# Bluear7878/Remote-Sensing-Vision-Language-Diffusion-Model

Measured on NVIDIA B200. Metric: stage2_denoise_steps_per_s_1024sq_cfg2, higher is better.
Workload: dtype bf16

## Files before the change

### remote-sensing-vision-language-diffusion-model_b200/csrc/attention.cu

```cuda
#include "common.cuh"

namespace b200sr {

static constexpr int ATT_BM = 128;
static constexpr int ATT_BN = 128;
static constexpr int ATT_D = 64;
static constexpr int ATT_THREADS = 320;
static constexpr int ATT_STAGES = 2;
static constexpr int ATT_TILE_BYTES = 128 * 64 * 2;
static constexpr int ATT_TMEM_COLS = 256;
static constexpr int ATT_COL_S = 0;
static constexpr int ATT_COL_P = 128;
static constexpr int ATT_COL_O = 192;
static constexpr int ATT_PART_FLOATS = 66 * 128;
static constexpr int ATT_WS_COUNTERS = 512;

struct AttnParams {
  int B, H, Nq, Nk;
  int q_col, k_col, v_col;
  __nv_bfloat16* out;
  long long ldo;
  float scale_log2;
  int causal;
  int n_qtiles, full_ctas, split, blocks_per_split;
  float* partials;
  unsigned int* counters;
#ifdef B200SR_ATT_TRACE
  long long* trace;
#endif
};

#ifdef B200SR_ATT_TRACE
static long long* g_att_trace = nullptr;
#define ATT_T(ev)                                                                                   \
  do {                                                                                              \
    if (p.trace != nullptr && lane == 0 && cta_lin < 4 && j < 64)                                   \
      p.trace[((cta_lin * 10 + warp) * 64 + j) * 8 + (ev)] = clock64();                             \
  } while (0)
__device__ __forceinline__ long long att_gtime() {
  long long t;
  asm volatile("mov.u64 %0, %globaltimer;" : "=l"(t));
  return t;
}
#define ATT_CTA(ev)                                                                                 \
  do {                                                                                              \
    if (p.trace != nullptr && threadIdx.x == 64 && cta_lin < 4096) {                                \
      p.trace[20480 + cta_lin * 3 + (ev)] = att_gtime();                                            \
      if ((ev) == 0) {                                                                              \
        uint32_t smid;                                                                              \
        asm volatile("mov.u32 %0, %smid;" : "=r"(smid));                                            \
        p.trace[20480 + cta_lin * 3 + 2] = smid;                                                    \
      }                                                                                             \
    }                                                                                               \
  } while (0)
#else
#define ATT_T(ev) do { } while (0)
#define ATT_CTA(ev) do { } while (0)
#endif

__device__ __forceinline__ void tmem_st32(uint32_t taddr, const uint32_t (&r)[32]) {
  asm volatile(
      "tcgen05.st.sync.aligned.32x32b.x32.b32 [%0], "
      "{%1, %2, %3, %4, %5, %6, %7, %8, %9, %10, %11, %12, %13, %14, %15, %16, "
      "%17, %18, %19, %20, %21, %22, %23, %24, %25, %26, %27, %28, %29, %30, %31, %32};" ::"r"(taddr),
      "r"(r[0]), "r"(r[1]), "r"(r[2]), "r"(r[3]), "r"(r[4]), "r"(r[5]), "r"(r[6]), "r"(r[7]), "r"(r[8]), "r"(r[9]),
      "r"(r[10]), "r"(r[11]), "r"(r[12]), "r"(r[13]), "r"(r[14]), "r"(r[15]), "r"(r[16]), "r"(r[17]), "r"(r[18]),
      "r"(r[19]), "r"(r[20]), "r"(r[21]), "r"(r[22]), "r"(r[23]), "r"(r[24]), "r"(r[25]), "r"(r[26]), "r"(r[27]),
      "r"(r[28]), "r"(r[29]), "r"(r[30]), "r"(r[31])
      : "memory");
}

__device__ __forceinline__ float ex2_approx(float x) {
  float y;
  asm("ex2.approx.ftz.f32 %0, %1;" : "=f"(y) : "f"(x));
  return y;
}

__global__ void __launch_bounds__(ATT_THREADS, 2)
attention_d64_kernel(const __grid_constant__ CUtensorMap tmQ, const __grid_constant__ CUtensorMap tmK,
                     const __grid_constant__ CUtensorMap tmV, const AttnParams p) {
  extern __shared__ __align__(1024) uint8_t smem_raw[];
  uint8_t* smem = reinterpret_cast<uint8_t*>((reinterpret_cast<uintptr_t>(smem_raw) + 1023) & ~uintptr_t(1023));
  uint8_t* sQ = smem;
  uint8_t* sKV = smem + ATT_TILE_BYTES;
  uint64_t* bars = reinterpret_cast<uint64_t*>(sKV + ATT_STAGES * 2 * ATT_TILE_BYTES);
  uint64_t* q_full = bars;
  uint64_t* kv_full = bars + 1;
  uint64_t* kv_empty = kv_full + ATT_STAGES;
  uint64_t* s_full = kv_empty + ATT_STAGES;
  uint64_t* p_full = s_full + 1;
  uint64_t* o_done = p_full + 1;
  uint32_t* tmem_slot = reinterpret_cast<uint32_t*>(o_done + 1);
  float* s_xch = reinterpret_cast<float*>(tmem_slot + 2);

  const int warp = threadIdx.x >> 5, lane = threadIdx.x & 31;
  int tile = blockIdx.x, jb0 = 0, split_idx = -1, tail_idx = 0;
  int nblk = (p.Nk + ATT_BN - 1) / ATT_BN;
  if (static_cast<int>(blockIdx.x) >= p.full_ctas) {
    const int t = blockIdx.x - p.full_ctas;
    tail_idx = t / p.split;
    split_idx = t - tail_idx * p.split;
    tile = p.full_ctas + tail_idx;
    jb0 = split_idx * p.blocks_per_split;
    nblk = min(nblk - jb0, p.blocks_per_split);
  }
  const int q0 = (tile % p.n_qtiles) * ATT_BM;
  const int h = (tile / p.n_qtiles) % p.H, b = tile / (p.n_qtiles * p.H);
#ifdef B200SR_ATT_TRACE
  const int cta_lin = blockIdx.x;
#endif
  ATT_CTA(0);

  if (warp == 0 && lane == 0) {
    tma_prefetch_desc(&tmQ);
    tma_prefetch_desc(&tmK);
    tma_prefetch_desc(&tmV);
    mbar_init(q_full, 1);
    for (int s = 0; s < ATT_STAGES; ++s) {
      mbar_init(&kv_full[s], 1);
      mbar_init(&kv_empty[s], 1);
    }
    mbar_init(s_full, 1);
    mbar_init(p_full, 8);
    mbar_init(o_done, 1);
    fence_barrier_init();
  }
  if (warp == 1) {
    tmem_alloc(tmem_slot, ATT_TMEM_COLS);
    tmem_relinquish();
  }
  tc_fence_before();
  __syncthreads();
  tc_fence_after();
  const uint32_t tmem = *tmem_slot;
  pdl_launch_dependents();

  if (warp == 0) {
    if (lane == 0) {
      pdl_wait();
      mbar_expect_tx(q_full, ATT_TILE_BYTES);
      tma_load_3d(sQ, &tmQ, q_full, p.q_col + h * ATT_D, q0, b);
      int stage = 0;
      uint32_t phase = 0;
      for (int j = 0; j < nblk; ++j) {
        mbar_wait(&kv_empty[stage], phase ^ 1);
        ATT_T(0);
        uint8_t* sK = sKV + stage * 2 * ATT_TILE_BYTES;
        uint8_t* sV = sK + ATT_TILE_BYTES;
        mbar_expect_tx(&kv_full[stage], 2 * ATT_TILE_BYTES);
        tma_load_3d(sK, &tmK, &kv_full[stage], p.k_col + h * ATT_D, (jb0 + j) * ATT_BN, b);
        tma_load_3d(sV, &tmV, &kv_full[stage], p.v_col + h * ATT_D, (jb0 + j) * ATT_BN, b);
        if (++stage == ATT_STAGES) {
          stage = 0;
          phase ^= 1;
        }
      }
    }
  } else if (warp == 1) {
    if (lane == 0) {
      const uint32_t idesc_s = umma_idesc_bf16_f32(ATT_BM, ATT_BN, 0, 0);
      const uint32_t idesc_o = umma_idesc_bf16_f32(ATT_BM, ATT_D, 0, 1);
      const uint64_t qdesc = umma_smem_desc_sw128(smem_u32(sQ), 16, 1024);
      mbar_wait(q_full, 0);
      int stage = 0;
      uint32_t phase = 0;
      mbar_wait(&kv_full[0], 0);
      tc_fence_after();
      {
        const uint64_t kdesc = umma_smem_desc_sw128(smem_u32(sKV), 16, 1024);
#pragma unroll
        for (int k = 0; k < ATT_D / 16; ++k) umma_ss(tmem + ATT_COL_S, qdesc + 2 * k, kdesc + 2 * k, idesc_s, k != 0);
        umma_commit(s_full);
      }
      for (int j = 0; j < nblk; ++j) {
        mbar_wait(p_full, j & 1);
        ATT_T(0);
        tc_fence_after();
        {
          const uint32_t sV = smem_u32(sKV + stage * 2 * ATT_TILE_BYTES + ATT_TILE_BYTES);
          const uint64_t vdesc = umma_smem_desc_sw128(sV, 1024, 1024);
#pragma unroll
          for (int k = 0; k < ATT_BN / 16; ++k) {
            umma_ts(tmem + ATT_COL_O, tmem + ATT_COL_P + 8 * k, vdesc + (2048 >> 4) * k, idesc_o, (j | k) != 0);
          }
          umma_commit(&kv_empty[stage]);
          if (j + 1 == nblk) umma_commit(o_done);
        }
        ATT_T(1);
        if (++stage == ATT_STAGES) {
          stage = 0;
          phase ^= 1;
        }
        if (j + 1 < nblk) {
          mbar_wait(&kv_full[stage], phase);
          ATT_T(2);
          tc_fence_after();
          const uint64_t kdesc = umma_smem_desc_sw128(smem_u32(sKV + stage * 2 * ATT_TILE_BYTES), 16, 1024);
#pragma unroll
          for (int k = 0; k < ATT_D / 16; ++k)
            umma_ss(tmem + ATT_COL_S, qdesc + 2 * k, kdesc + 2 * k, idesc_s, k != 0);
          umma_commit(s_full);
          ATT_T(3);
        }
      }
    }
  } else {
    const int sub = warp & 3;
    const int half = (warp - 2) >> 2;
    const int r = sub * 32 + lane;
    const uint32_t lane_base = static_cast<uint32_t>(sub * 32) << 16;
    float m_used = -INFINITY;
    float l = 0.f;
    for (int j = 0; j < nblk; ++j) {
      mbar_wait(s_full, j & 1);
      ATT_T(0);
      tc_fence_after();
      float s[64];
#pragma unroll
      for (int c = 0; c < 2; ++c) {
        uint32_t a[32];
        tmem_ld32(tmem + lane_base + ATT_COL_S + half * 64 + c * 32, a);
#pragma unroll
        for (int i = 0; i < 32; ++i) s[c * 32 + i] = __uint_as_float(a[i]);
      }
      tmem_ld_wait();
      ATT_T(1);
      int kv_left = p.Nk - (jb0 + j) * ATT_BN - half * 64;
      if (p.causal) kv_left = min(kv_left, q0 + r + 1 - (jb0 + j) * ATT_BN - half * 64);
      if (kv_left < 64) {
#pragma unroll
        for (int i = 0; i < 64; ++i)
          if (i >= kv_left) s[i] = -INFINITY;
      }
      float mx = s[0];
#pragma unroll
      for (int i = 1; i < 64; ++i) mx = fmaxf(mx, s[i]);
      float* xch = s_xch + (j & 1) * 256;
      xch[half * 128 + r] = mx;
      asm volatile("bar.sync 1, 256;" ::: "memory");
      ATT_T(2);
      mx = fmaxf(mx, xch[(half ^ 1) * 128 + r]) * p.scale_log2;
      const bool grow = mx > m_used + 8.0f;
      if (j == 0) {
        m_used = mx;
      } else if (__any_sync(0xffffffffu, grow)) {
        float alpha = 1.0f;
        if (grow) {
          alpha = ex2_approx(m_used - mx);
          m_used = mx;
          l *= alpha;
        }
        uint32_t o[32];
        tmem_ld32(tmem + lane_base + ATT_COL_O + half * 32, o);
        tmem_ld_wait();
#pragma unroll
        for (int i = 0; i < 32; ++i) o[i] = __float_as_uint(__uint_as_float(o[i]) * alpha);
        tmem_st32(tmem + lane_base + ATT_COL_O + half * 32, o);
      }
      float sum0 = 0.f, sum1 = 0.f;
      uint32_t pk[32];
#pragma unroll
      for (int i = 0; i < 32; ++i) {
        const float e0 = ex2_approx(fmaf(s[2 * i], p.scale_log2, -m_used));
        const float e1 = ex2_approx(fmaf(s[2 * i + 1], p.scale_log2, -m_used));
        sum0 += e0;
        sum1 += e1;
        pk[i] = pack_bf16x2(e0, e1);
      }
      ATT_T(3);
      tmem_st32(tmem + lane_base + ATT_COL_P + half * 32, pk);
      l += sum0 + sum1;
      tmem_st_wait();
      ATT_T(4);
      tc_fence_before();
      __syncwarp();
      if (lane == 0) mbar_arrive(p_full);
      ATT_T(5);
    }
    float* xch = s_xch + (nblk & 1) * 256;
    xch[half * 128 + r] = l;
    asm volatile("bar.sync 1, 256;" ::: "memory");
    l += xch[(half ^ 1) * 128 + r];
    mbar_wait(o_done, 0);
    tc_fence_after();
    const int q = q0 + r;
    uint32_t o[32];
    tmem_ld32(tmem + lane_base + ATT_COL_O + half * 32, o);
    tmem_ld_wait();
    bool write_out = true;
    if (split_idx >= 0) {
      float* part = p.partials + (static_cast<size_t>(tail_idx) * p.split + split_idx) * ATT_PART_FLOATS;
#pragma unroll
      for (int i = 0; i < 32; ++i) part[(half * 32 + i) * 128 + r] = __uint_as_float(o[i]);
      if (half == 0) {
        part[64 * 128 + r] = m_used;
        part[65 * 128 + r] = l;
      }
      __threadfence();
      asm volatile("bar.sync 1, 256;" ::: "memory");
      if (threadIdx.x == 64) {
        const unsigned int prev = atomicAdd(&p.counters[tail_idx], 1u);
        tmem_slot[1] = (prev == static_cast<unsigned int>(p.split) - 1u) ? 1u : 0u;
        __threadfence();
      }
      asm volatile("bar.sync 1, 256;" ::: "memory");
      write_out = tmem_slot[1] != 0u;
      if (write_out) {
        const float* base = p.partials + static_cast<size_t>(tail_idx) * p.split * ATT_PART_FLOATS;
        float m_all = -INFINITY;
        for (int s2 = 0; s2 < p.split; ++s2) m_all = fmaxf(m_all, __ldcg(base + s2 * ATT_PART_FLOATS + 64 * 128 + r));
        float acc[32];
#pragma unroll
        for (int i = 0; i < 32; ++i) acc[i] = 0.f;
        l = 0.f;
        for (int s2 = 0; s2 < p.split; ++s2) {
          const float* ps = base + s2 * ATT_PART_FLOATS;
          const float w = ex2_approx(__ldcg(ps + 64 * 128 + r) - m_all);
          l = fmaf(w, __ldcg(ps + 65 * 128 + r), l);
#pragma unroll
          for (int i = 0; i < 32; ++i) acc[i] = fmaf(w, __ldcg(ps + (half * 32 + i) * 128 + r), acc[i]);
        }
#pragma unroll
        for (int i = 0; i < 32; ++i) o[i] = __float_as_uint(acc[i]);
        if (threadIdx.x == 64) p.counters[tail_idx] = 0u;
      }
    }
    const float inv_l = 1.0f / l;
    if (write_out && q < p.Nq) {
      __nv_bfloat16* dst = p.out + (static_cast<long long>(b) * p.Nq + q) * p.ldo + h * ATT_D + half * 32;
#pragma unroll
      for (int v = 0; v < 4; ++v) {
        uint4 u;
        u.x = pack_bf16x2(__uint_as_float(o[v * 8 + 0]) * inv_l, __uint_as_float(o[v * 8 + 1]) * inv_l);
        u.y = pack_bf16x2(__uint_as_float(o[v * 8 + 2]) * inv_l, __uint_as_float(o[v * 8 + 3]) * inv_l);
        u.z = pack_bf16x2(__uint_as_float(o[v * 8 + 4]) * inv_l, __uint_as_float(o[v * 8 + 5]) * inv_l);
        u.w = pack_bf16x2(__uint_as_float(o[v * 8 + 6]) * inv_l, __uint_as_float(o[v * 8 + 7]) * inv_l);
        reinterpret_cast<uint4*>(dst)[v] = u;
      }
    }
  }

  ATT_CTA(1);
  tc_fence_before();
  __syncthreads();
  tc_fence_after();
  if (warp == 1) tmem_dealloc(tmem, ATT_TMEM_COLS);
}

static int make_map3(CUtensorMap* m, const void* base, long long ld, int rows, int batch, int width_cols) {
  uint64_t dims[3] = {static_cast<uint64_t>(width_cols), static_cast<uint64_t>(rows), static_cast<uint64_t>(batch)};
  uint64_t strides[2] = {static_cast<uint64_t>(ld) * 2, static_cast<uint64_t>(rows) * ld * 2};
  uint32_t box[3] = {ATT_D, 128, 1};
  return make_tmap_bf16(m, base, 3, dims, strides, box);
}

struct AttnPlan {
  int n_qtiles, tiles, full, tail, split, blocks_per_split;
  size_t workspace_bytes;
};

static AttnPlan attention_plan(int B, int H, int Nq, int Nk) {
  AttnPlan a;
  a.n_qtiles = (Nq + ATT_BM - 1) / ATT_BM;
  a.tiles = B * H * a.n_qtiles;
  const int nblk = (Nk + ATT_BN - 1) / ATT_BN;
  const int slots = 2 * num_sms();
  a.split = 1;
  a.blocks_per_split = nblk;
  a.full = a.tiles;
  a.tail = 0;
  if (slots <= 0) {
    a.workspace_bytes = 0;
    return a;
  }
  a.full = (a.tiles / slots) * slots;
  a.tail = a.tiles - a.full;
  if (a.tail > 0 && a.tail <= ATT_WS_COUNTERS) {
    int s = 1;
    while (s * 2 <= nblk && a.tail * s * 2 <= slots && s * 2 <= 4) s *= 2;
    if (s > 1) {
      a.blocks_per_split = (nblk + s - 1) / s;
      a.split = (nblk + a.blocks_per_split - 1) / a.blocks_per_split;
    }
  }
  if (a.split == 1) {
    a.full = a.tiles;
    a.tail = 0;
  }
  a.workspace_bytes = a.tail == 0 ? 0
                                  : ATT_WS_COUNTERS * sizeof(unsigned int) +
                                        static_cast<size_t>(a.tail) * a.split * ATT_PART_FLOATS * sizeof(float);
  return a;
}

size_t attention_d64_workspace_bytes(int B, int H, int Nq, int Nk) {
  if (B <= 0 || H <= 0 || Nq <= 0 || Nk <= 0) return 0;
  return attention_plan(B, H, Nq, Nk).workspace_bytes;
}

int attention_d64(const void* q, long long ldq, int q_col, const void* k, long long ldk, int k_col, const void* v,
                  long long ldv, int v_col, void* out, long long ldo, int B, int H, int Nq, int Nk, float scale,
                  int causal, void* workspace, cudaStream_t stream) {
  if (B <= 0 || H <= 0 || Nq <= 0 || Nk <= 0) return B200SR_EINVAL;
  if (causal && (Nq != Nk || Nk > ATT_BN)) return B200SR_EINVAL;
  if ((ldq % 8) || (ldk % 8) || (ldv % 8) || (ldo % 8) || (q_col % 8) || (k_col % 8) || (v_col % 8))
    return B200SR_EINVAL;
  if (q_col + H * ATT_D > ldq || k_col + H * ATT_D > ldk || v_col + H * ATT_D > ldv || H * ATT_D > ldo)
    return B200SR_EINVAL;
  const AttnPlan plan = attention_plan(B, H, Nq, Nk);
  if (plan.workspace_bytes != 0 && workspace == nullptr) return B200SR_EINVAL;
  CUtensorMap tmQ, tmK, tmV;
  int rc = make_map3(&tmQ, q, ldq, Nq, B, static_cast<int>(ldq));
  if (rc) return rc;
  rc = make_map3(&tmK, k, ldk, Nk, B, static_cast<int>(ldk));
  if (rc) return rc;
  rc = make_map3(&tmV, v, ldv, Nk, B, static_cast<int>(ldv));
  if (rc) return rc;
  AttnParams p;
  p.B = B;
  p.H = H;
  p.Nq = Nq;
  p.Nk = Nk;
  p.q_col = q_col;
  p.k_col = k_col;
  p.v_col = v_col;
  p.out = reinterpret_cast<__nv_bfloat16*>(out);
  p.ldo = ldo;
  p.scale_log2 = scale * 1.4426950408889634f;
  p.causal = causal;
  p.n_qtiles = plan.n_qtiles;
  p.full_ctas = plan.full;
  p.split = plan.split;
  p.blocks_per_split = plan.blocks_per_split;
  p.counters = reinterpret_cast<unsigned int*>(workspace);
  p.partials = reinterpret_cast<float*>(reinterpret_cast<unsigned int*>(workspace) + ATT_WS_COUNTERS);
#ifdef B200SR_ATT_TRACE
  p.trace = g_att_trace;
#endif
  const size_t smem_bytes = ATT_TILE_BYTES * (1 + 2 * ATT_STAGES) + 1024 + 128 + 2048;
  static bool attr_set[64] = {false};
  if (first_use_on_device(attr_set)) {
    if (cudaFuncSetAttribute(attention_d64_kernel, cudaFuncAttributeMaxDynamicSharedMemorySize,
                             static_cast<int>(smem_bytes)) != cudaSuccess)
      return B200SR_ELAUNCH;
  }
  dim3 grid(plan.full + plan.tail * plan.split);
  return launch_k(attention_d64_kernel, grid, dim3(ATT_THREADS), smem_bytes, stream, 1, tmQ, tmK, tmV, p) == cudaSuccess
             ? B200SR_OK
             : B200SR_ELAUNCH;
}

}

#ifdef B200SR_ATT_TRACE
extern "C" void b200sr_debug_set_attn_trace(void* p) { b200sr::g_att_trace = reinterpret_cast<long long*>(p); }
#endif
```

Measured before the change: 38.20.

## Process two Q tiles per CTA with ping-pong softmax and shared K/V stages

Each CTA now handles a pair of adjacent 128-row query tiles that share every K/V block. Each tile gets its own 256-column TMEM region and its own 4-warp softmax group, and a polling MMA issuer interleaves QK and PV for both units so one unit's tensor-core work overlaps the other's softmax. K/V staging grows to three stages and the cross-half max exchange through shared memory is removed, since each thread now owns a full 128-wide row. The kernel drops to one CTA per SM with 512 TMEM columns, so it loses inter-CTA overlap, risks register pressure from the 128-float row, and the grid shrinks, which may hurt tail balance.

```diff
diff --git a/remote-sensing-vision-language-diffusion-model_b200/csrc/attention.cu b/remote-sensing-vision-language-diffusion-model_b200/csrc/attention.cu
--- a/remote-sensing-vision-language-diffusion-model_b200/csrc/attention.cu
+++ b/remote-sensing-vision-language-diffusion-model_b200/csrc/attention.cu
@@ -6,9 +6,10 @@
 static constexpr int ATT_BN = 128;
 static constexpr int ATT_D = 64;
 static constexpr int ATT_THREADS = 320;
-static constexpr int ATT_STAGES = 2;
+static constexpr int ATT_STAGES = 3;
 static constexpr int ATT_TILE_BYTES = 128 * 64 * 2;
-static constexpr int ATT_TMEM_COLS = 256;
+static constexpr int ATT_TMEM_COLS = 512;
+static constexpr int ATT_UNIT_COLS = 256;
 static constexpr int ATT_COL_S = 0;
 static constexpr int ATT_COL_P = 128;
 static constexpr int ATT_COL_O = 192;
@@ -22,7 +23,7 @@
   long long ldo;
   float scale_log2;
   int causal;
-  int n_qtiles, full_ctas, split, blocks_per_split;
+  int n_qtiles, full_tiles, tiles, full_ctas, split, blocks_per_split;
   float* partials;
   unsigned int* counters;
 #ifdef B200SR_ATT_TRACE
@@ -30,12 +31,44 @@
 #endif
 };
 
+__host__ __device__ inline int att_pairs(int lo, int hi, int nq) {
+  if (lo >= hi) return 0;
+  const int head_end = (lo / nq + 1) * nq;
+  const int a0 = (hi < head_end ? hi : head_end) - lo;
+  const int rest = hi - lo - a0;
+  return (a0 + 1) / 2 + (rest / nq) * ((nq + 1) / 2) + (rest % nq + 1) / 2;
+}
+__device__ __forceinline__ int att_pair_at(int c, int lo, int hi, int nq, bool& has1) {
+  const int a0 = min(hi, (lo / nq + 1) * nq) - lo;
+  const int c0 = (a0 + 1) / 2;
+  int t, head_end;
+  if (c < c0) {
+    t = lo + 2 * c;
+    head_end = lo + a0;
+  } else {
+    c -= c0;
+    const int cph = (nq + 1) / 2;
+    const int g = c / cph;
+    t = lo + a0 + g * nq + 2 * (c - g * cph);
+    head_end = min(hi, lo + a0 + (g + 1) * nq);
+  }
+  has1 = t + 1 < head_end;
+  return t;
+}
+
 #ifdef B200SR_ATT_TRACE
 static long long* g_att_trace = nullptr;
+static constexpr int ATT_TRACE_EV = 16;
+static constexpr int ATT_TRACE_CTA_OFF = 4 * 10 * 64 * ATT_TRACE_EV;
 #define ATT_T(ev)                                                                                   \
   do {                                                                                              \
     if (p.trace != nullptr && lane == 0 && cta_lin < 4 && j < 64)                                   \
-      p.trace[((cta_lin * 10 + warp) * 64 + j) * 8 + (ev)] = clock64();                             \
+      p.trace[((cta_lin * 10 + warp) * 64 + j) * ATT_TRACE_EV + (ev)] = clock64();                  \
+  } while (0)
+#define ATT_TV(ev, val)                                                                             \
+  do {                                                                                              \
+    if (p.trace != nullptr && lane == 0 && cta_lin < 4 && j < 64)                                   \
+      p.trace[((cta_lin * 10 + warp) * 64 + j) * ATT_TRACE_EV + (ev)] = (val);                      \
   } while (0)
 __device__ __forceinline__ long long att_gtime() {
   long long t;
@@ -45,17 +78,25 @@
 #define ATT_CTA(ev)                                                                                 \
   do {                                                                                              \
     if (p.trace != nullptr && threadIdx.x == 64 && cta_lin < 4096) {                                \
-      p.trace[20480 + cta_lin * 3 + (ev)] = att_gtime();                                            \
+      p.trace[ATT_TRACE_CTA_OFF + cta_lin * 3 + (ev)] = att_gtime();                                \
       if ((ev) == 0) {                                                                              \
         uint32_t smid;                                                                              \
         asm volatile("mov.u32 %0, %smid;" : "=r"(smid));                                            \
-        p.trace[20480 + cta_lin * 3 + 2] = smid;                                                    \
+        p.trace[ATT_TRACE_CTA_OFF + cta_lin * 3 + 2] = smid;                                        \
       }                                                                                             \
     }                                                                                               \
   } while (0)
+#define ATT_MMA_ISSUE(stmt)                                                                         \
+  do {                                                                                              \
+    const long long t_i = clock64();                                                                \
+    stmt;                                                                                           \
+    busy += clock64() - t_i;                                                                        \
+  } while (0)
 #else
 #define ATT_T(ev) do { } while (0)
+#define ATT_TV(ev, val) do { } while (0)
 #define ATT_CTA(ev) do { } while (0)
+#define ATT_MMA_ISSUE(stmt) stmt
 #endif
 
 __device__ __forceinline__ void tmem_st32(uint32_t taddr, const uint32_t (&r)[32]) {
@@ -76,36 +117,48 @@
   return y;
 }
 
-__global__ void __launch_bounds__(ATT_THREADS, 2)
+__device__ __forceinline__ void bar_sync_unit(int u) {
+  if (u == 0)
+    asm volatile("bar.sync 1, 128;" ::: "memory");
+  else
+    asm volatile("bar.sync 2, 128;" ::: "memory");
+}
+
+__global__ void __launch_bounds__(ATT_THREADS, 1)
 attention_d64_kernel(const __grid_constant__ CUtensorMap tmQ, const __grid_constant__ CUtensorMap tmK,
                      const __grid_constant__ CUtensorMap tmV, const AttnParams p) {
   extern __shared__ __align__(1024) uint8_t smem_raw[];
   uint8_t* smem = reinterpret_cast<uint8_t*>((reinterpret_cast<uintptr_t>(smem_raw) + 1023) & ~uintptr_t(1023));
   uint8_t* sQ = smem;
-  uint8_t* sKV = smem + ATT_TILE_BYTES;
+  uint8_t* sKV = smem + 2 * ATT_TILE_BYTES;
   uint64_t* bars = reinterpret_cast<uint64_t*>(sKV + ATT_STAGES * 2 * ATT_TILE_BYTES);
   uint64_t* q_full = bars;
   uint64_t* kv_full = bars + 1;
   uint64_t* kv_empty = kv_full + ATT_STAGES;
   uint64_t* s_full = kv_empty + ATT_STAGES;
-  uint64_t* p_full = s_full + 1;
-  uint64_t* o_done = p_full + 1;
-  uint32_t* tmem_slot = reinterpret_cast<uint32_t*>(o_done + 1);
-  float* s_xch = reinterpret_cast<float*>(tmem_slot + 2);
+  uint64_t* s_free = s_full + 2;
+  uint64_t* p_full = s_free + 2;
+  uint64_t* pv_done = p_full + 2;
+  uint32_t* tmem_slot = reinterpret_cast<uint32_t*>(pv_done + 2);
+  uint32_t* last_flag = tmem_slot + 1;
 
   const int warp = threadIdx.x >> 5, lane = threadIdx.x & 31;
-  int tile = blockIdx.x, jb0 = 0, split_idx = -1, tail_idx = 0;
+  bool has1;
+  int tile0, jb0 = 0, split_idx = -1;
   int nblk = (p.Nk + ATT_BN - 1) / ATT_BN;
-  if (static_cast<int>(blockIdx.x) >= p.full_ctas) {
-    const int t = blockIdx.x - p.full_ctas;
-    tail_idx = t / p.split;
-    split_idx = t - tail_idx * p.split;
-    tile = p.full_ctas + tail_idx;
+  if (static_cast<int>(blockIdx.x) < p.full_ctas) {
+    tile0 = att_pair_at(blockIdx.x, 0, p.full_tiles, p.n_qtiles, has1);
+  } else {
+    const int c = blockIdx.x - p.full_ctas;
+    const int pair = c / p.split;
+    split_idx = c - pair * p.split;
+    tile0 = att_pair_at(pair, p.full_tiles, p.tiles, p.n_qtiles, has1);
     jb0 = split_idx * p.blocks_per_split;
     nblk = min(nblk - jb0, p.blocks_per_split);
   }
-  const int q0 = (tile % p.n_qtiles) * ATT_BM;
-  const int h = (tile / p.n_qtiles) % p.H, b = tile / (p.n_qtiles * p.H);
+  const int nunits = has1 ? 2 : 1;
+  const int q00 = (tile0 % p.n_qtiles) * ATT_BM;
+  const int h = (tile0 / p.n_qtiles) % p.H, b = tile0 / (p.n_qtiles * p.H);
 #ifdef B200SR_ATT_TRACE
   const int cta_lin = blockIdx.x;
 #endif
@@ -120,9 +173,12 @@
       mbar_init(&kv_full[s], 1);
       mbar_init(&kv_empty[s], 1);
     }
-    mbar_init(s_full, 1);
-    mbar_init(p_full, 8);
-    mbar_init(o_done, 1);
+    for (int u = 0; u < 2; ++u) {
+      mbar_init(&s_full[u], 1);
+      mbar_init(&s_free[u], 4);
+      mbar_init(&p_full[u], 4);
+      mbar_init(&pv_done[u], 1);
+    }
     fence_barrier_init();
   }
   if (warp == 1) {
@@ -138,13 +194,13 @@
   if (warp == 0) {
     if (lane == 0) {
       pdl_wait();
-      mbar_expect_tx(q_full, ATT_TILE_BYTES);
-      tma_load_3d(sQ, &tmQ, q_full, p.q_col + h * ATT_D, q0, b);
+      mbar_expect_tx(q_full, nunits * ATT_TILE_BYTES);
+      for (int u = 0; u < nunits; ++u)
+        tma_load_3d(sQ + u * ATT_TILE_BYTES, &tmQ, q_full, p.q_col + h * ATT_D, q00 + u * ATT_BM, b);
       int stage = 0;
       uint32_t phase = 0;
       for (int j = 0; j < nblk; ++j) {
         mbar_wait(&kv_empty[stage], phase ^ 1);
-        ATT_T(0);
         uint8_t* sK = sKV + stage * 2 * ATT_TILE_BYTES;
         uint8_t* sV = sK + ATT_TILE_BYTES;
         mbar_expect_tx(&kv_full[stage], 2 * ATT_TILE_BYTES);
@@ -160,182 +216,235 @@
     if (lane == 0) {
       const uint32_t idesc_s = umma_idesc_bf16_f32(ATT_BM, ATT_BN, 0, 0);
       const uint32_t idesc_o = umma_idesc_bf16_f32(ATT_BM, ATT_D, 0, 1);
-      const uint64_t qdesc = umma_smem_desc_sw128(smem_u32(sQ), 16, 1024);
+#ifdef B200SR_ATT_TRACE
+      long long busy = 0;
+#endif
+      auto issue_qk = [&](int u, int stage) {
+        const uint64_t qdesc = umma_smem_desc_sw128(smem_u32(sQ + u * ATT_TILE_BYTES), 16, 1024);
+        const uint64_t kdesc = umma_smem_desc_sw128(smem_u32(sKV + stage * 2 * ATT_TILE_BYTES), 16, 1024);
+#pragma unroll
+        for (int k = 0; k < ATT_D / 16; ++k)
+          umma_ss(tmem + u * ATT_UNIT_COLS + ATT_COL_S, qdesc + 2 * k, kdesc + 2 * k, idesc_s, k != 0);
+        umma_commit(&s_full[u]);
+      };
+      auto issue_pv = [&](int u, int stage, int j) {
+        const uint64_t vdesc =
+            umma_smem_desc_sw128(smem_u32(sKV + stage * 2 * ATT_TILE_BYTES + ATT_TILE_BYTES), 1024, 1024);
+        const uint32_t tu = tmem + u * ATT_UNIT_COLS;
+#pragma unroll
+        for (int k = 0; k < ATT_BN / 16; ++k) {
+          umma_ts(tu + ATT_COL_O, tu + ATT_COL_P + 8 * k, vdesc + (2048 >> 4) * k, idesc_o, (j | k) != 0);
+        }
+        umma_commit(&pv_done[u]);
+      };
       mbar_wait(q_full, 0);
-      int stage = 0;
-      uint32_t phase = 0;
       mbar_wait(&kv_full[0], 0);
       tc_fence_after();
-      {
-        const uint64_t kdesc = umma_smem_desc_sw128(smem_u32(sKV), 16, 1024);
-#pragma unroll
-        for (int k = 0; k < ATT_D / 16; ++k) umma_ss(tmem + ATT_COL_S, qdesc + 2 * k, kdesc + 2 * k, idesc_s, k != 0);
-        umma_commit(s_full);
-      }
-      for (int j = 0; j < nblk; ++j) {
-        mbar_wait(p_full, j & 1);
-        ATT_T(0);
-        tc_fence_after();
-        {
-          const uint32_t sV = smem_u32(sKV + stage * 2 * ATT_TILE_BYTES + ATT_TILE_BYTES);
-          const uint64_t vdesc = umma_smem_desc_sw128(sV, 1024, 1024);
-#pragma unroll
-          for (int k = 0; k < ATT_BN / 16; ++k) {
-            umma_ts(tmem + ATT_COL_O, tmem + ATT_COL_P + 8 * k, vdesc + (2048 >> 4) * k, idesc_o, (j | k) != 0);
+      for (int u = 0; u < nunits; ++u) issue_qk(u, 0);
+      int qk_next[2] = {1, 1}, pv_next[2] = {0, 0};
+      if (nunits == 1) qk_next[1] = pv_next[1] = nblk;
+      int kv_ready = 1, freed = 0;
+#if B200SR_HANG_GUARD
+      long long t_idle = 0;
+      uint32_t idle = 0;
+#endif
+      while (freed < nblk) {
+        bool progress = false;
+        if (kv_ready < nblk && mbar_test_wait(&kv_full[kv_ready % ATT_STAGES], (kv_ready / ATT_STAGES) & 1)) {
+          const int j = kv_ready;
+          ATT_T(0);
+          ++kv_ready;
+          progress = true;
+        }
+#pragma unroll
+        for (int u = 0; u < 2; ++u) {
+          const int jp = pv_next[u];
+          if (jp < qk_next[u] && mbar_test_wait(&p_full[u], jp & 1)) {
+            tc_fence_after();
+            ATT_MMA_ISSUE(issue_pv(u, jp % ATT_STAGES, jp));
+            const int j = jp;
+            ATT_T(2 + 2 * u);
+            pv_next[u] = jp + 1;
+            progress = true;
           }
-          umma_commit(&kv_empty[stage]);
-          if (j + 1 == nblk) umma_commit(o_done);
-        }
-        ATT_T(1);
-        if (++stage == ATT_STAGES) {
-          stage = 0;
-          phase ^= 1;
-        }
-        if (j + 1 < nblk) {
-          mbar_wait(&kv_full[stage], phase);
-          ATT_T(2);
-          tc_fence_after();
-          const uint64_t kdesc = umma_smem_desc_sw128(smem_u32(sKV + stage * 2 * ATT_TILE_BYTES), 16, 1024);
-#pragma unroll
-          for (int k = 0; k < ATT_D / 16; ++k)
-            umma_ss(tmem + ATT_COL_S, qdesc + 2 * k, kdesc + 2 * k, idesc_s, k != 0);
-          umma_commit(s_full);
-          ATT_T(3);
-        }
+          const int jq = qk_next[u];
+          if (jq < kv_ready && mbar_test_wait(&s_free[u], (jq - 1) & 1)) {
+            tc_fence_after();
+            ATT_MMA_ISSUE(issue_qk(u, jq % ATT_STAGES));
+            const int j = jq;
+            ATT_T(1 + 2 * u);
+            qk_next[u] = jq + 1;
+            progress = true;
+          }
+        }
+        while (freed < min(pv_next[0], pv_next[1])) {
+          umma_commit(&kv_empty[freed % ATT_STAGES]);
+          const int j = freed;
+          ATT_T(5);
+          ATT_TV(8, busy);
+          ++freed;
+          progress = true;
+        }
+#if B200SR_HANG_GUARD
+        if (progress) {
+          idle = 0;
+        } else if (++idle == 1024u) {
+          t_idle = clock64();
+        } else if (idle > 1024u && (idle & 1023u) == 0 && clock64() - t_idle > 8000000000LL) {
+          __trap();
+        }
+#endif
       }
     }
   } else {
-    const int sub = warp & 3;
-    const int half = (warp - 2) >> 2;
-    const int r = sub * 32 + lane;
-    const uint32_t lane_base = static_cast<uint32_t>(sub * 32) << 16;
-    float m_used = -INFINITY;
-    float l = 0.f;
-    for (int j = 0; j < nblk; ++j) {
-      mbar_wait(s_full, j & 1);
-      ATT_T(0);
+    const int u = (warp - 2) >> 2;
+    const int quad = warp & 3;
+    const int r = quad * 32 + lane;
+    const uint32_t tu = tmem + (static_cast<uint32_t>(quad * 32) << 16) + u * ATT_UNIT_COLS;
+    const int q0 = q00 + u * ATT_BM;
+    if (u < nunits) {
+      float m_used = -INFINITY;
+      float l = 0.f;
+      for (int j = 0; j < nblk; ++j) {
+        mbar_wait(&s_full[u], j & 1);
+        ATT_T(0);
+        tc_fence_after();
+        float s[128];
+#pragma unroll
+        for (int c = 0; c < 4; ++c) {
+          uint32_t a[32];
+          tmem_ld32(tu + ATT_COL_S + c * 32, a);
+#pragma unroll
+          for (int i = 0; i < 32; ++i) s[c * 32 + i] = __uint_as_float(a[i]);
+        }
+        tmem_ld_wait();
+        tc_fence_before();
+        __syncwarp();
+        if (lane == 0) mbar_arrive(&s_free[u]);
+        ATT_T(1);
+        int kv_left = p.Nk - (jb0 + j) * ATT_BN;
+        if (p.causal) kv_left = min(kv_left, q0 + r + 1 - (jb0 + j) * ATT_BN);
+        if (kv_left < ATT_BN) {
+#pragma unroll
+          for (int i = 0; i < ATT_BN; ++i)
+            if (i >= kv_left) s[i] = -INFINITY;
+        }
+        float mx0 = s[0], mx1 = s[1], mx2 = s[2], mx3 = s[3];
+#pragma unroll
+        for (int i = 4; i < ATT_BN; i += 4) {
+          mx0 = fmaxf(mx0, s[i]);
+          mx1 = fmaxf(mx1, s[i + 1]);
+          mx2 = fmaxf(mx2, s[i + 2]);
+          mx3 = fmaxf(mx3, s[i + 3]);
+        }
+        const float mx = fmaxf(fmaxf(mx0, mx1), fmaxf(mx2, mx3)) * p.scale_log2;
+        ATT_T(2);
+        const bool grow = mx > m_used + 8.0f;
+        const bool rescale = j != 0 && __any_sync(0xffffffffu, grow);
+        float alpha = 1.0f;
+        if (j == 0) {
+          m_used = mx;
+        } else {
+          if (grow) {
+            alpha = ex2_approx(m_used - mx);
+            m_used = mx;
+            l *= alpha;
+          }
+          mbar_wait(&pv_done[u], (j - 1) & 1);
+          tc_fence_after();
+        }
+        ATT_T(3);
+        float sum[4] = {0.f, 0.f, 0.f, 0.f};
+#pragma unroll
+        for (int c = 0; c < 4; ++c) {
+          uint32_t pk[16];
+#pragma unroll
+          for (int i = 0; i < 16; ++i) {
+            const float e0 = ex2_approx(fmaf(s[c * 32 + 2 * i], p.scale_log2, -m_used));
+            const float e1 = ex2_approx(fmaf(s[c * 32 + 2 * i + 1], p.scale_log2, -m_used));
+            sum[(c >> 1) * 2] += e0;
+            sum[(c >> 1) * 2 + 1] += e1;
+            pk[i] = pack_bf16x2(e0, e1);
+          }
+          tmem_st16(tu + ATT_COL_P + c * 16, pk);
+        }
+        l += (sum[0] + sum[1]) + (sum[2] + sum[3]);
+        if (rescale) {
+#pragma unroll
+          for (int c = 0; c < 2; ++c) {
+            uint32_t o[32];
+            tmem_ld32(tu + ATT_COL_O + c * 32, o);
+            tmem_ld_wait();
+#pragma unroll
+            for (int i = 0; i < 32; ++i) o[i] = __float_as_uint(__uint_as_float(o[i]) * alpha);
+            tmem_st32(tu + ATT_COL_O + c * 32, o);
+          }
+        }
+        ATT_T(4);
+        tmem_st_wait();
+        tc_fence_before();
+        __syncwarp();
+        if (lane == 0) mbar_arrive(&p_full[u]);
+        ATT_T(5);
+      }
+      mbar_wait(&pv_done[u], (nblk - 1) & 1);
       tc_fence_after();
-      float s[64];
+      const int q = q0 + r;
+      float o[64];
 #pragma unroll
       for (int c = 0; c < 2; ++c) {
         uint32_t a[32];
-        tmem_ld32(tmem + lane_base + ATT_COL_S + half * 64 + c * 32, a);
-#pragma unroll
-        for (int i = 0; i < 32; ++i) s[c * 32 + i] = __uint_as_float(a[i]);
+        tmem_ld32(tu + ATT_COL_O + c * 32, a);
+        tmem_ld_wait();
+#pragma unroll
+        for (int i = 0; i < 32; ++i) o[c * 32 + i] = __uint_as_float(a[i]);
       }
-      tmem_ld_wait();
-      ATT_T(1);
-      int kv_left = p.Nk - (jb0 + j) * ATT_BN - half * 64;
-      if (p.causal) kv_left = min(kv_left, q0 + r + 1 - (jb0 + j) * ATT_BN - half * 64);
-      if (kv_left < 64) {
-#pragma unroll
-        for (int i = 0; i < 64; ++i)
-          if (i >= kv_left) s[i] = -INFINITY;
-      }
-      float mx = s[0];
-#pragma unroll
-      for (int i = 1; i < 64; ++i) mx = fmaxf(mx, s[i]);
-      float* xch = s_xch + (j & 1) * 256;
-      xch[half * 128 + r] = mx;
-      asm volatile("bar.sync 1, 256;" ::: "memory");
-      ATT_T(2);
-      mx = fmaxf(mx, xch[(half ^ 1) * 128 + r]) * p.scale_log2;
-      const bool grow = mx > m_used + 8.0f;
-      if (j == 0) {
-        m_used = mx;
-      } else if (__any_sync(0xffffffffu, grow)) {
-        float alpha = 1.0f;
-        if (grow) {
-          alpha = ex2_approx(m_used - mx);
-          m_used = mx;
-          l *= alpha;
-        }
-        uint32_t o[32];
-        tmem_ld32(tmem + lane_base + ATT_COL_O + half * 32, o);
-        tmem_ld_wait();
-#pragma unroll
-        for (int i = 0; i < 32; ++i) o[i] = __float_as_uint(__uint_as_float(o[i]) * alpha);
-        tmem_st32(tmem + lane_base + ATT_COL_O + half * 32, o);
-      }
-      float sum0 = 0.f, sum1 = 0.f;
-      uint32_t pk[32];
-#pragma unroll
-      for (int i = 0; i < 32; ++i) {
-        const float e0 = ex2_approx(fmaf(s[2 * i], p.scale_log2, -m_used));
-        const float e1 = ex2_approx(fmaf(s[2 * i + 1], p.scale_log2, -m_used));
-        sum0 += e0;
-        sum1 += e1;
-        pk[i] = pack_bf16x2(e0, e1);
-      }
-      ATT_T(3);
-      tmem_st32(tmem + lane_base + ATT_COL_P + half * 32, pk);
-      l += sum0 + sum1;
-      tmem_st_wait();
-      ATT_T(4);
-      tc_fence_before();
-      __syncwarp();
-      if (lane == 0) mbar_arrive(p_full);
-      ATT_T(5);
-    }
-    float* xch = s_xch + (nblk & 1) * 256;
-    xch[half * 128 + r] = l;
-    asm volatile("bar.sync 1, 256;" ::: "memory");
-    l += xch[(half ^ 1) * 128 + r];
-    mbar_wait(o_done, 0);
-    tc_fence_after();
-    const int q = q0 + r;
-    uint32_t o[32];
-    tmem_ld32(tmem + lane_base + ATT_COL_O + half * 32, o);
-    tmem_ld_wait();
-    bool write_out = true;
-    if (split_idx >= 0) {
-      float* part = p.partials + (static_cast<size_t>(tail_idx) * p.split + split_idx) * ATT_PART_FLOATS;
-#pragma unroll
-      for (int i = 0; i < 32; ++i) part[(half * 32 + i) * 128 + r] = __uint_as_float(o[i]);
-      if (half == 0) {
+      bool write_out = true;
+      if (split_idx >= 0) {
+        const int tail_idx = tile0 + u - p.full_tiles;
+        float* part = p.partials + (static_cast<size_t>(tail_idx) * p.split + split_idx) * ATT_PART_FLOATS;
+#pragma unroll
+        for (int i = 0; i < 64; ++i) part[i * 128 + r] = o[i];
         part[64 * 128 + r] = m_used;
         part[65 * 128 + r] = l;
+        __threadfence();
+        bar_sync_unit(u);
+        if (r == 0) {
+          const unsigned int prev = atomicAdd(&p.counters[tail_idx], 1u);
+          last_flag[u] = (prev == static_cast<unsigned int>(p.split) - 1u) ? 1u : 0u;
+          __threadfence();
+        }
+        bar_sync_unit(u);
+        write_out = last_flag[u] != 0u;
+        if (write_out) {
+          const float* base = p.partials + static_cast<size_t>(tail_idx) * p.split * ATT_PART_FLOATS;
+          float m_all = -INFINITY;
+          for (int s2 = 0; s2 < p.split; ++s2) m_all = fmaxf(m_all, __ldcg(base + s2 * ATT_PART_FLOATS + 64 * 128 + r));
+#pragma unroll
+          for (int i = 0; i < 64; ++i) o[i] = 0.f;
+          l = 0.f;
+          for (int s2 = 0; s2 < p.split; ++s2) {
+            const float* ps = base + s2 * ATT_PART_FLOATS;
+            const float w = ex2_approx(__ldcg(ps + 64 * 128 + r) - m_all);
+            l = fmaf(w, __ldcg(ps + 65 * 128 + r), l);
+#pragma unroll
+            for (int i = 0; i < 64; ++i) o[i] = fmaf(w, __ldcg(ps + i * 128 + r), o[i]);
+          }
+          if (r == 0) p.counters[tail_idx] = 0u;
+        }
       }
-      __threadfence();
-      asm volatile("bar.sync 1, 256;" ::: "memory");
-      if (threadIdx.x == 64) {
-        const unsigned int prev = atomicAdd(&p.counters[tail_idx], 1u);
-        tmem_slot[1] = (prev == static_cast<unsigned int>(p.split) - 1u) ? 1u : 0u;
-        __threadfence();
-      }
-      asm volatile("bar.sync 1, 256;" ::: "memory");
-      write_out = tmem_slot[1] != 0u;
-      if (write_out) {
-        const float* base = p.partials + static_cast<size_t>(tail_idx) * p.split * ATT_PART_FLOATS;
-        float m_all = -INFINITY;
-        for (int s2 = 0; s2 < p.split; ++s2) m_all = fmaxf(m_all, __ldcg(base + s2 * ATT_PART_FLOATS + 64 * 128 + r));
-        float acc[32];
-#pragma unroll
-        for (int i = 0; i < 32; ++i) acc[i] = 0.f;
-        l = 0.f;
-        for (int s2 = 0; s2 < p.split; ++s2) {
-          const float* ps = base + s2 * ATT_PART_FLOATS;
-          const float w = ex2_approx(__ldcg(ps + 64 * 128 + r) - m_all);
-          l = fmaf(w, __ldcg(ps + 65 * 128 + r), l);
-#pragma unroll
-          for (int i = 0; i < 32; ++i) acc[i] = fmaf(w, __ldcg(ps + (half * 32 + i) * 128 + r), acc[i]);
-        }
-#pragma unroll
-        for (int i = 0; i < 32; ++i) o[i] = __float_as_uint(acc[i]);
-        if (threadIdx.x == 64) p.counters[tail_idx] = 0u;
-      }
-    }
-    const float inv_l = 1.0f / l;
-    if (write_out && q < p.Nq) {
-      __nv_bfloat16* dst = p.out + (static_cast<long long>(b) * p.Nq + q) * p.ldo + h * ATT_D + half * 32;
-#pragma unroll
-      for (int v = 0; v < 4; ++v) {
-        uint4 u;
-        u.x = pack_bf16x2(__uint_as_float(o[v * 8 + 0]) * inv_l, __uint_as_float(o[v * 8 + 1]) * inv_l);
-        u.y = pack_bf16x2(__uint_as_float(o[v * 8 + 2]) * inv_l, __uint_as_float(o[v * 8 + 3]) * inv_l);
-        u.z = pack_bf16x2(__uint_as_float(o[v * 8 + 4]) * inv_l, __uint_as_float(o[v * 8 + 5]) * inv_l);
-        u.w = pack_bf16x2(__uint_as_float(o[v * 8 + 6]) * inv_l, __uint_as_float(o[v * 8 + 7]) * inv_l);
-        reinterpret_cast<uint4*>(dst)[v] = u;
+      const float inv_l = 1.0f / l;
+      if (write_out && q < p.Nq) {
+        __nv_bfloat16* dst = p.out + (static_cast<long long>(b) * p.Nq + q) * p.ldo + h * ATT_D;
+#pragma unroll
+        for (int v = 0; v < 8; ++v) {
+          uint4 w;
+          w.x = pack_bf16x2(o[v * 8 + 0] * inv_l, o[v * 8 + 1] * inv_l);
+          w.y = pack_bf16x2(o[v * 8 + 2] * inv_l, o[v * 8 + 3] * inv_l);
+          w.z = pack_bf16x2(o[v * 8 + 4] * inv_l, o[v * 8 + 5] * inv_l);
+          w.w = pack_bf16x2(o[v * 8 + 6] * inv_l, o[v * 8 + 7] * inv_l);
+          reinterpret_cast<uint4*>(dst)[v] = w;
+        }
       }
     }
   }
@@ -429,7 +538,9 @@
   p.scale_log2 = scale * 1.4426950408889634f;
   p.causal = causal;
   p.n_qtiles = plan.n_qtiles;
-  p.full_ctas = plan.full;
+  p.full_tiles = plan.full;
+  p.tiles = plan.tiles;
+  p.full_ctas = att_pairs(0, plan.full, plan.n_qtiles);
   p.split = plan.split;
   p.blocks_per_split = plan.blocks_per_split;
   p.counters = reinterpret_cast<unsigned int*>(workspace);
@@ -437,14 +548,14 @@
 #ifdef B200SR_ATT_TRACE
   p.trace = g_att_trace;
 #endif
-  const size_t smem_bytes = ATT_TILE_BYTES * (1 + 2 * ATT_STAGES) + 1024 + 128 + 2048;
+  const size_t smem_bytes = ATT_TILE_BYTES * (2 + 2 * ATT_STAGES) + 1024 + 256;
   static bool attr_set[64] = {false};
   if (first_use_on_device(attr_set)) {
     if (cudaFuncSetAttribute(attention_d64_kernel, cudaFuncAttributeMaxDynamicSharedMemorySize,
                              static_cast<int>(smem_bytes)) != cudaSuccess)
       return B200SR_ELAUNCH;
   }
-  dim3 grid(plan.full + plan.tail * plan.split);
+  dim3 grid(p.full_ctas + att_pairs(plan.full, plan.tiles, plan.n_qtiles) * plan.split);
   return launch_k(attention_d64_kernel, grid, dim3(ATT_THREADS), smem_bytes, stream, 1, tmQ, tmK, tmV, p) == cudaSuccess
              ? B200SR_OK
              : B200SR_ELAUNCH;
```

Result: faster. 39.30 (median of 6 runs) (+2.9%).
